# febos/SQUARNA

Measured on AMD Instinct MI355X. Metric: sequences/sec (SRtest150, single-sequence mode), higher is better.
Workload: dtype f64; 1 GPU; SRtest150 if=qf c=nobpp poollim=1000; 8 independent batches in flight per GPU (sq_fold_concurrent, one stream set each), each holding the 219-record set 12 time(s); a step folds all of them; the batches run free inside the timed region (every batch is folded `steps` times back to back, no barrier between the steps: sq_fold_concurrent_n); batches_in_flight=8, sets_per_batch=12, hw_queues=4

## Files before the change

squarna_amd/csrc/sq_lsap.h:

```cpp
#pragma once
#include "sq_match.h"

enum SqLsapForm {
    SQ_LSAP_A,
    SQ_LSAP_B,
    SQ_LSAP_C
};

struct SqLsapLayout {
    double *cost;
    double *u, *v, *spc;
    int32_t *path, *col4row, *row4col, *remaining;
    uint8_t *SR, *SC;
    double *wts;
    uint32_t *mask;
    uint16_t *rowstart;
    uint16_t *pre;
    uint16_t *cids;
    int nw;
    size_t sparse_off;
    size_t lds_end, scratch_end;
};

SQ_HD static inline SqLsapLayout sq_lsap_carve(char *scratch, char *lds, SqLsapForm form, int n, int m)
{
    SqLsapLayout L;
    const size_t N = (size_t)n, M = (size_t)m;
    L.nw = (n + 31) >> 5;
    size_t os = 0, ol = 0;
    sq_take(scratch, os, L.cost, N * N);
    const bool glob = form == SQ_LSAP_C;
    char *const vb = glob ? scratch + os : lds;
    size_t ov = 0;
    sq_take(vb, ov, L.u, N); sq_take(vb, ov, L.v, N); sq_take(vb, ov, L.spc, N);
    sq_take(vb, ov, L.path, N); sq_take(vb, ov, L.col4row, N); sq_take(vb, ov, L.row4col, N); sq_take(vb, ov, L.remaining, N);
    sq_take(vb, ov, L.SR, N); sq_take(vb, ov, L.SC, N);
    if (glob) os += ov;
    ol = ov;
    sq_take(lds, ol, L.wts, M, 16);
    L.sparse_off = (size_t)(reinterpret_cast<char *>(L.wts) - lds);
    sq_take(lds, ol, L.mask, N * L.nw);
    sq_take(lds, ol, L.rowstart, N + 1);
    sq_take(lds, ol, L.pre, N * L.nw, 4);
    sq_take(lds, ol, L.cids, 2 * M, 4);
    L.lds_end = ol; L.scratch_end = os;
    return L;
}

SQ_HD static inline size_t sq_lsap_vec_bytes(int n) { return sq_lsap_carve(nullptr, nullptr, SQ_LSAP_A, n, 0).sparse_off; }
SQ_HD static inline size_t sq_lsap_sparse_bytes(int n, int m)
{
    const SqLsapLayout L = sq_lsap_carve(nullptr, nullptr, SQ_LSAP_A, n, m);
    return L.lds_end - L.sparse_off + 16;
}
SQ_HD static inline size_t sq_lsap_lds_bytes(int n, int m) { return sq_lsap_vec_bytes(n) + sq_lsap_sparse_bytes(n, m) + 64; }
SQ_HD static inline size_t sq_lsap_scratch_bytes(int n) { return sq_lsap_carve(nullptr, nullptr, SQ_LSAP_C, n, 0).scratch_end + 64; }

SQ_HD static inline SqLsapForm sq_lsap_form(int n, int m, size_t lds_bytes)
{
    const bool vec_lds = sq_lsap_vec_bytes(n) + 64 <= lds_bytes;
    const bool mat_lds = vec_lds && m < 32767 && sq_lsap_lds_bytes(n, m) <= lds_bytes;
    return mat_lds ? SQ_LSAP_A : vec_lds ? SQ_LSAP_B : SQ_LSAP_C;
}

struct SqLsapSyncNone {
    SQ_HD void operator()() const {}
    SQ_HD void after_lane0(bool) const {}
};

template <int W, class Sync, class Coop>
SQ_HD_INLINE void sq_lsap_run(const SqLsapLayout &L, SqLsapForm form, int n, int m, const SqMatchEdge *edges, int lane, Sync sync, Coop coop)
{
    const double inf = __builtin_huge_val();
    const bool mat_lds = form == SQ_LSAP_A;
    const int nw = L.nw;
    double *const cost = L.cost, *const u = L.u, *const v = L.v, *const spc = L.spc, *const wts = L.wts;
    int32_t *const path = L.path, *const col4row = L.col4row, *const row4col = L.row4col, *const remaining = L.remaining;
    uint8_t *const SR = L.SR, *const SC = L.SC;
    uint32_t *const mask = L.mask;
    uint16_t *const rowstart = L.rowstart, *const pre = L.pre, *const cids = L.cids;

    if (mat_lds) {
        for (int q = lane; q < n * nw; q += W) mask[q] = 0u;
    } else {
        for (size_t q = lane; q < (size_t)n * n; q += W) cost[q] = 0.0;
    }
    for (int q = lane; q < n; q += W) { u[q] = 0.0; v[q] = 0.0; path[q] = -1; col4row[q] = -1; row4col[q] = -1; }
    sync();
    if (mat_lds) {
        for (int e = lane; e < m; e += W) {
            const SqMatchEdge ed = edges[e];
            wts[e] = ed.weight;
            coop.or_u32(&mask[ed.v * nw + (ed.w >> 5)], 1u << (ed.w & 31));
            coop.or_u32(&mask[ed.w * nw + (ed.v >> 5)], 1u << (ed.v & 31));
        }
        sync();
        const int per = (n + W - 1) / W, r0 = lane * per < n ? lane * per : n, r1 = r0 + per < n ? r0 + per : n;
        int mine = 0;
        for (int r = r0; r < r1; r++) {
            int acc = 0;
            for (int w = 0; w < nw; w++) { pre[r * nw + w] = (uint16_t)acc; acc += __builtin_popcount(mask[r * nw + w]); }
            mine += acc;
        }
        int total = 0;
        int run = coop.excl_scan(mine, total);
        for (int r = r0; r < r1; r++) {
            rowstart[r] = (uint16_t)run;
            run += (int)pre[r * nw + nw - 1] + __builtin_popcount(mask[r * nw + nw - 1]);
        }
        if (lane == W - 1) rowstart[n] = (uint16_t)total;
        sync();
        for (int e = lane; e < m; e += W) {
            const SqMatchEdge ed = edges[e];
            const int a = ed.v, c = ed.w;
            cids[rowstart[a] + pre[a * nw + (c >> 5)] + __builtin_popcount(mask[a * nw + (c >> 5)] & ((1u << (c & 31)) - 1u))] = (uint16_t)e;
            cids[rowstart[c] + pre[c * nw + (a >> 5)] + __builtin_popcount(mask[c * nw + (a >> 5)] & ((1u << (a & 31)) - 1u))] = (uint16_t)e;
        }
    } else {
        for (int e = lane; e < m; e += W) {
            const SqMatchEdge ed = edges[e];
            cost[(size_t)ed.v * n + ed.w] = -ed.weight;
            cost[(size_t)ed.w * n + ed.v] = -ed.weight;
        }
    }
    sync();

    for (int cur = 0; cur < n; cur++) {
        for (int q = lane; q < n; q += W) { remaining[q] = n - q - 1; SR[q] = 0; SC[q] = 0; spc[q] = inf; }
        int i = cur, sink = -1, nrem = n;
        double minval = 0.0;
        sync();
        while (sink == -1) {
            const double ui = u[i];
            const int rs_i = mat_lds ? (int)rowstart[i] : 0;
            double lowest = inf;
            int first = -1, lastun = -1;
            for (int it0 = 0; it0 < nrem; it0 += 3 * W) {
                int jj[3]; bool have[3];
                SQ_UNROLL
                for (int t = 0; t < 3; t++) { const int it = it0 + W * t + lane; have[t] = it < nrem; jj[t] = remaining[have[t] ? it : 0]; }
                uint32_t wd[3]; int pw[3], r4[3]; double vj[3], spj[3], cij[3];
                SQ_UNROLL
                for (int t = 0; t < 3; t++) {
                    const int j = jj[t];
                    vj[t] = v[j]; spj[t] = spc[j]; r4[t] = row4col[j];
                    if (mat_lds) { wd[t] = mask[i * nw + (j >> 5)]; pw[t] = (int)pre[i * nw + (j >> 5)]; cij[t] = 0.0; }
                    else { wd[t] = 0u; pw[t] = 0; cij[t] = cost[(size_t)i * n + j]; }
                }
                if (mat_lds) {
                    int cid[3];
                    SQ_UNROLL
                    for (int t = 0; t < 3; t++) {
                        const int j = jj[t];
                        const bool nz = (wd[t] >> (j & 31)) & 1u;
                        cid[t] = nz ? (int)cids[rs_i + pw[t] + __builtin_popcount(wd[t] & ((1u << (j & 31)) - 1u))] : -1;
                    }
                    SQ_UNROLL
                    for (int t = 0; t < 3; t++) cij[t] = cid[t] >= 0 ? -wts[cid[t]] : 0.0;
                }
                SQ_UNROLL
                for (int t = 0; t < 3; t++) {
                    if (!have[t]) continue;
                    const int it = it0 + W * t + lane, j = jj[t];
                    const double r = minval + cij[t] - ui - vj[t];
                    double sp = spj[t];
                    if (r < sp) { path[j] = i; spc[j] = r; sp = r; }
                    const bool un = r4[t] == -1;
                    if (sp < lowest) { lowest = sp; first = it; lastun = un ? it : -1; }
                    else if (sp == lowest && un) lastun = it;
                }
            }
            double mn = lowest;
            coop.min_plain(mn);
            int f = (lowest == mn && first >= 0) ? first : 0x7fffffff;
            coop.min_i32(f);
            int lu = -((lowest == mn) ? lastun : -1);
            coop.min_i32(lu);
            lu = -lu;
            minval = mn;
            if (mn == inf) { if (lane == 0) SR[i] = 1; sink = -2; break; }
            const int index = lu >= 0 ? lu : f;
            const int j = remaining[index], lastj = remaining[nrem - 1];
            const int owner = row4col[j];
            sync();
            if (lane == 0) { SR[i] = 1; SC[j] = 1; remaining[index] = lastj; }
            nrem--;
            if (owner == -1) sink = j; else i = owner;
            sync.after_lane0(form == SQ_LSAP_C);
        }
        if (sink < 0) break;
        if (lane == 0) u[cur] += minval;
        for (int q = lane; q < n; q += W) {
            if (SR[q] && q != cur) u[q] += minval - spc[col4row[q]];
            if (SC[q]) v[q] -= minval - spc[q];
        }
        sync();
        if (lane == 0) {
            int j = sink;
            for (;;) {
                const int i2 = path[j];
                row4col[j] = i2;
                const int t = col4row[i2]; col4row[i2] = j; j = t;
                if (i2 == cur) break;
            }
        }
        sync();
    }
}
```

squarna_amd/csrc/sq_match.hip:

```cpp
#include <hip/hip_runtime.h>
#include <stdint.h>
#include <math.h>
#include <stdlib.h>
#include <stdio.h>
#include "sq_match.h"
#include "sq_switches.h"
#include "sq_hostflag.h"
#include <vector>
#include <algorithm>
#include "sq_blossom.h"
#include "sq_algo_plan.h"

struct SqLsapBlockSync {
    __device__ void operator()() const { __syncthreads(); }
    __device__ void after_lane0(bool glob) const
    {
        if (glob) __builtin_amdgcn_fence(__ATOMIC_RELEASE, "workgroup");
        __syncthreads();
        if (glob) __builtin_amdgcn_fence(__ATOMIC_ACQUIRE, "workgroup");
    }
};

extern "C" __global__ __launch_bounds__(64) void sq_lsap_kernel(const SqMatchJob *jobs, const SqMatchEdge *edges,
                                                                char *scratch, int32_t *col4row_out, int lds_bytes)
{
    extern __shared__ __attribute__((aligned(16))) char lsap_lds[];
    const SqMatchJob jb = jobs[blockIdx.x];
    const int n = jb.n, m = jb.nedges, lane = threadIdx.x;
    if (n <= 0) return;
    const SqLsapForm form = sq_lsap_form(n, m, (size_t)lds_bytes);
    const SqLsapLayout L = sq_lsap_carve(scratch + jb.scratch_off, lsap_lds, form, n, m);
    sq_lsap_run<64>(L, form, n, m, edges + jb.edge_off, lane, SqLsapBlockSync(), SqCoopWave());
    for (int q = lane; q < n; q += 64) col4row_out[jb.out_off + q] = L.col4row[q];
}

extern "C" __global__ __launch_bounds__(256) void sq_nussinov_kernel(const SqMatchJob *jobs, const SqMatchEdge *edges,
                                                                     const uint8_t *codes, char *scratch,
                                                                     int32_t *pairs_out, int32_t *count_out, int by_pad)
{
    const SqMatchJob jb = jobs[blockIdx.x];
    const int n = jb.n, tid = threadIdx.x, nthr = blockDim.x;
    int32_t *const my_count = count_out + (by_pad ? jb.pad : (int)blockIdx.x);
    if (n < 2) { if (tid == 0) *my_count = 0; return; }
    sq_nussinov_run(sq_nuss_carve(scratch + jb.scratch_off, n, jb.nedges), n, jb.nedges, edges + jb.edge_off, codes + jb.pos_off,
                    pairs_out + 2 * (size_t)jb.out_off, my_count, tid, nthr, [] { __syncthreads(); }, SqCoopWave());
}

template <class Sync>
__device__ __forceinline__ void sq_mwm_one(SqBlossom &bl, char *lds_base, char *wlds, size_t lds_bytes, const SqMatchJob *jp, int row,
                                           const SqMatchEdge *edges, char *scratch, int32_t *mate_out, uint32_t *job_flags,
                                           uint32_t stamp, int lane, Sync wsync)
{
    auto publish = [&]() {
        if (job_flags) {
            const int nw = jp->n > 0 ? 2 * jp->n + 2 : 2;
            sq_host_write_flush(mate_out + jp->out_off + (lane < nw ? nw - 1 - lane : 0));
        }
        wsync();
        if (job_flags && lane == 0) job_flags[row] = stamp;
    };
    const int n = jp->n, m = jp->nedges;
    if (n <= 0) { if (lane == 0) { mate_out[jp->out_off] = 0; mate_out[jp->out_off + 1] = 0; } publish(); return; }
#ifdef SQ_MWM_PROF
    const long long _c0 = clock64(), _w0 = wall_clock64();
#endif
    const size_t ebytes = ((size_t)m * sizeof(SqMatchEdge) + 15) & ~(size_t)15;
    char *gscratch = scratch + jp->scratch_off;
    const bool all_lds = SqBlossom::scratch_bytes(n, m, 1) + ebytes + 16 <= lds_bytes;
    const bool hot_lds = !all_lds && SqBlossom::hot_bytes(n, m, 2) + 16 <= lds_bytes;
    if (all_lds) {
        SqMatchEdge *le = reinterpret_cast<SqMatchEdge *>(wlds);
        for (int e = lane; e < m; e += 64) le[e] = edges[jp->edge_off + e];
        wsync();
#ifdef SQ_MWM_PROF
        const long long _w1 = wall_clock64();
#endif
        if (lane == 0) { bl.init(n, m, le, wlds + ebytes, 1, false); bl.origin = lds_base; }
        wsync();
#ifdef SQ_MWM_PROF
        const long long _w2 = wall_clock64();
#endif
        bl.template build_csr<1>(lane, 64, wsync, SqCoopWave());
#ifdef SQ_MWM_PROF
        const long long _w3 = wall_clock64();
#endif
        bl.template run<1>(lane, 64, wsync, SqCoopWave(), lds_base);
#ifdef SQ_MWM_PROF
        if (lane == 0 && n >= 140) printf("mwm outside: edge load %.0f us, init %.0f, csr %.0f, run %.0f\n", (_w1 - _w0) * 0.01, (_w2 - _w1) * 0.01, (_w3 - _w2) * 0.01, (wall_clock64() - _w3) * 0.01);
#endif
    } else if (hot_lds) {
        if (lane == 0) {
            char *cold = gscratch;
            bl.init(n, m, edges + jp->edge_off, wlds, 2, false, cold, cold + ((SqBlossom::cold_bytes(n, m, 2) + 15) & ~(size_t)15));
            bl.origin = lds_base;
        }
        wsync();
        bl.template build_csr<2>(lane, 64, wsync, SqCoopWave());
        bl.template run<2>(lane, 64, wsync, SqCoopWave(), lds_base);
    }
    if (all_lds || hot_lds) {
        wsync();
        if (!bl.error) {
            for (int q = lane; q < n; q += 64) { mate_out[jp->out_off + q] = bl.mate[q]; mate_out[jp->out_off + n + q] = bl.mord[q]; }
            if (lane == 0) { mate_out[jp->out_off + 2 * n] = bl.stat_pass; mate_out[jp->out_off + 2 * n + 1] = bl.stat_event; }
#ifdef SQ_MWM_PROF
            if (lane == 0 && n >= 140) {
                const long long dc = clock64() - _c0, dw = wall_clock64() - _w0;
                printf("mwm clock: %lld shader cycles in %.0f us -> %.0f MHz\n", dc, dw * 0.01, (double)dc / (dw * 0.01));
            }
#endif
            publish();
            return;
        }
        wsync();
    }
    if (lane == 0) bl.init(n, m, edges + jp->edge_off, gscratch, 0, false);
    wsync();
    bl.template build_csr<0>(lane, 64, wsync, SqCoopWave());
    bl.template run<0>(lane, 64, wsync, SqCoopWave(), nullptr);
    wsync();
    for (int q = lane; q < n; q += 64) { mate_out[jp->out_off + q] = bl.error ? -2 : bl.mate[q]; mate_out[jp->out_off + n + q] = bl.mord[q]; }
    if (lane == 0) { mate_out[jp->out_off + 2 * n] = bl.stat_pass; mate_out[jp->out_off + 2 * n + 1] = bl.stat_event; }
    publish();
}

extern "C" __global__ __launch_bounds__(512, 4) void sq_mwm_kernel(const SqMatchJob *jobs, const int32_t *bin_head,
                                                                const SqMatchEdge *edges, char *scratch, int32_t *mate_out,
                                                                uint32_t *job_flags, uint32_t stamp)
{
    extern __shared__ __attribute__((aligned(16))) char mwm_lds[];
    const int wave = threadIdx.x >> 6, lane = threadIdx.x & 63;
    int row = bin_head[blockIdx.x];
    for (int k = 0; k < wave && row >= 0; k++) row = jobs[row].next;
    if (row < 0) return;
    auto wsync = [] { __builtin_amdgcn_fence(__ATOMIC_SEQ_CST, "workgroup"); __builtin_amdgcn_wave_barrier(); };
    const SqMatchJob *jp = jobs + row;
    const size_t hdr = (sizeof(SqBlossom) + 15) & ~(size_t)15;
    SqBlossom &bl = *reinterpret_cast<SqBlossom *>(mwm_lds + jp->lds_off);
    const size_t lds_bytes = (size_t)jp->lds_bytes > hdr ? (size_t)jp->lds_bytes - hdr : 0;
    sq_mwm_one(bl, mwm_lds, mwm_lds + jp->lds_off + hdr, lds_bytes, jp, row, edges, scratch, mate_out, job_flags, stamp, lane, wsync);
}

extern "C" __global__ __launch_bounds__(64) void sq_mwm_single_kernel(const SqMatchJob *jobs, const SqMatchEdge *edges, char *scratch,
                                                                     int32_t *mate_out, int lds_bytes, uint32_t *job_flags,
                                                                     uint32_t stamp)
{
    __shared__ SqBlossom bl;
    extern __shared__ __attribute__((aligned(16))) char mwm_lds[];
    sq_mwm_one(bl, mwm_lds, mwm_lds, (size_t)lds_bytes, jobs + blockIdx.x, (int)blockIdx.x, edges, scratch, mate_out, job_flags, stamp,
               (int)threadIdx.x, [] { __syncthreads(); });
}

extern "C" __global__ void sq_flag_kernel(uint32_t *flag, uint32_t value)
{
    sq_host_write_flush(flag);
    *flag = value;
}

SqAlgoKnobs sq_algo_knobs(int lsap_classes)
{
    const SqTuning &tu = sq_tuning();
    SqAlgoKnobs kn;
    kn.mwm_classes = tu.mwm_classes; kn.lsap_classes = lsap_classes;
    kn.mwm_bin_waves = tu.mwm_bin_waves; kn.mwm_bin_bytes = tu.mwm_bin_bytes; kn.mwm_all_cap = tu.mwm_all_cap;
    kn.mwm_nolds = tu.mwm_nolds; kn.nuss_threads = tu.nuss_threads;
    return kn;
}

int sq_launch_matching(int algo, const SqMatchJob *h_jobs, int nj, const SqMatchJob *jobs, const SqMatchEdge *edges,
                       size_t nedges, SqMatchEdge *dev_edges, char *d_scr, int32_t *out, int32_t *cnt,
                       const uint8_t *codes, uint32_t *job_flags, uint32_t flag_val, hipStream_t st,
                       SqMatchJob *jobs_rw, int32_t *bin_head, int inflight, const SqAlgoKnobs &kn, bool dump)
{
    int maxn = 0, maxm = 0;
    for (int q = 0; q < nj; q++) { maxn = maxn > h_jobs[q].n ? maxn : h_jobs[q].n; maxm = maxm > h_jobs[q].nedges ? maxm : h_jobs[q].nedges; }
    if (algo == 4) {
        const SqLsapLds P = sq_lsap_launch_lds(h_jobs, nj);
        if (P.need > 64 * 1024) sq_max_dynamic_lds((const void *)sq_lsap_kernel, (int)SQ_LSAP_LDS_CAP);
        hipLaunchKernelGGL(sq_lsap_kernel, dim3(nj), dim3(64), P.lds, st, jobs, edges, d_scr, out, (int)P.lds);
    } else if (algo == 2) {
        const int nthr = sq_nussinov_threads(h_jobs, nj, maxn, inflight, kn);
        hipLaunchKernelGGL(sq_nussinov_kernel, dim3(nj), dim3(nthr), 0, st, jobs, edges, codes, d_scr, out, cnt, jobs_rw ? 1 : 0);
    } else {
        const SqMwmPlan P = sq_mwm_plan(h_jobs, jobs_rw, nj, bin_head, inflight, kn, dump);
        const size_t lds = P.lds;
        sq_max_dynamic_lds((const void *)sq_mwm_kernel, 156 * 1024);
        if (!P.all_in_lds && dev_edges != edges) {
            hipError_t e = hipMemcpyAsync(dev_edges, edges, nedges * sizeof(SqMatchEdge), hipMemcpyHostToDevice, st);
            if (e != hipSuccess) return (int)e;
            edges = dev_edges;
        }
        if (P.waves == 1) {
            sq_max_dynamic_lds((const void *)sq_mwm_single_kernel, 156 * 1024);
            const size_t one = lds > sq_blossom_hdr() ? lds - sq_blossom_hdr() : 0;
            hipLaunchKernelGGL(sq_mwm_single_kernel, dim3(nj), dim3(64), one, st, jobs, edges, d_scr, out, (int)one, job_flags, flag_val);
        } else
            hipLaunchKernelGGL(sq_mwm_kernel, dim3(P.nbins), dim3(64 * P.waves), lds, st, jobs, bin_head, edges, d_scr, out, job_flags, flag_val);
    }
    return (int)hipGetLastError();
}
```

squarna_amd/csrc/sq_nussinov.h:

```cpp
#pragma once
#include "sq_match.h"

struct SqNussLayout {
    double *cs;
    int32_t *ck;
    int32_t *col_off, *cursor;
    double *D;
    int32_t *K;
    uint8_t *has;
    int32_t *cur, *nxt;
    size_t lists_end, lists_room;
    size_t end;
};

SQ_HD static inline SqNussLayout sq_nuss_carve(char *scratch, int n, int m)
{
    SqNussLayout L;
    const size_t N = (size_t)n, M = (size_t)m;
    size_t o = 0;
    sq_take(scratch, o, L.cs, M); sq_take(scratch, o, L.ck, M); sq_take(scratch, o, L.col_off, N + 1); sq_take(scratch, o, L.cursor, N);
    L.lists_end = o;
    o = L.lists_room = N * N * sizeof(double);
    sq_take(scratch, o, L.D, N * N);
    sq_take(scratch, o, L.K, N * N);
    sq_take(scratch, o, L.has, (N * N + 15) & ~(size_t)15);
    sq_take(scratch, o, L.cur, 2 * (N + 2)); sq_take(scratch, o, L.nxt, 2 * (N + 2));
    L.end = o;
    return L;
}

static inline size_t sq_nussinov_scratch_bytes(int n) { return sq_nuss_carve(nullptr, n, 0).end + 64; }

template <class Sync, class Coop>
SQ_HD_INLINE void sq_nussinov_run(const SqNussLayout &L, int n, int m, const SqMatchEdge *edges, const uint8_t *cd, int32_t *out,
                                  int32_t *count, int tid, int nthr, Sync sync, Coop coop)
{
    double *const cs = L.cs;
    int32_t *const ck = L.ck, *const col_off = L.col_off, *const cursor = L.cursor;
    uint8_t *const has = L.has;
    for (size_t q = tid; q < (size_t)n * n; q += nthr) has[q] = 0;
    for (int q = tid; q < n; q += nthr) L.D[(size_t)q * n + q] = 0.0;
    for (int q = tid; q <= n; q += nthr) col_off[q] = 0;
    sync();
    for (int e = tid; e < m; e += nthr) coop.add_i32(&col_off[edges[e].w + 1], 1);
    sync();
    if (tid == 0) for (int j = 0; j < n; j++) col_off[j + 1] += col_off[j];
    sync();
    for (int q = tid; q < n; q += nthr) cursor[q] = col_off[q];
    sync();
    for (int e = tid; e < m; e += nthr) {
        const SqMatchEdge ed = edges[e];
        const int pos = coop.fetch_add_i32(&cursor[ed.w], 1);
        ck[pos] = ed.v; cs[pos] = -ed.weight;
    }
    sync();
    for (int j = tid; j < n; j += nthr) {
        const int a = col_off[j], b = col_off[j + 1];
        for (int x = a + 1; x < b; x++) {
            const int kk = ck[x]; const double vv = cs[x];
            int y = x - 1;
            while (y >= a && ck[y] > kk) { ck[y + 1] = ck[y]; cs[y + 1] = cs[y]; y--; }
            ck[y + 1] = kk; cs[y + 1] = vv;
        }
    }
    sync();
    double *const Dc = L.D;
    int32_t *const Kc = L.K;
    for (int j = 1; j < n; j++) {
        const int x0 = col_off[j], x1 = col_off[j + 1];
        const double *const dprevcol = Dc + (size_t)(j - 1) * n;
        for (int i = tid; i < j; i += nthr) {
            int bestk = -1; double best = 1e9;
            for (int x = x0; x < x1; x += 4) {
                int kk[4]; double d1[4], d2[4], cw[4]; bool ok[4];
                SQ_UNROLL
                for (int t = 0; t < 4; t++) { const int k = ck[x + t < x1 ? x + t : x]; kk[t] = x + t < x1 ? k : 0x7fffffff; }
                SQ_UNROLL
                for (int t = 0; t < 4; t++) {
                    ok[t] = kk[t] >= i && kk[t] < j - 1;
                    d1[t] = 0.0; d2[t] = 0.0; cw[t] = 0.0;
                    if (ok[t]) {
                        if (kk[t] > i) d1[t] = Dc[(size_t)(kk[t] - 1) * n + i];
                        d2[t] = dprevcol[kk[t] + 1];
                        cw[t] = cs[x + t];
                    }
                }
                SQ_UNROLL
                for (int t = 0; t < 4; t++)
                    if (ok[t]) {
                        const double sc = d1[t] + d2[t] + cw[t];
                        if (sc < best) { bestk = kk[t]; best = sc; }
                    }
                if (kk[3] >= j - 1) break;
            }
            const double dprev = dprevcol[i];
            const bool take = best <= dprev;
            Kc[(size_t)j * n + i] = take ? bestk : -2;
            Dc[(size_t)j * n + i] = take ? best : dprev;
        }
        sync();
    }
    if (tid == 0) {
        const int minloop = 3;
        int32_t *const cur = L.cur, *const nxt = L.nxt;
        uint8_t *inq = has;
        int qn = 1, np = 0;
        cur[0] = 0; cur[1] = n - 1;
        auto sep = [&](int p) { return cd[p] == 26 || cd[p] == 27; };
        auto anysep = [&](int a, int b) { for (int x = a; x < b; x++) if (x >= 0 && x < n && sep(x)) return true; return false; };
        while (qn) {
            int nn = 0;
            for (int t = 0; t < qn; t++) {
                const int i = cur[2 * t], j = cur[2 * t + 1];
                if (i < 0 || j < 0 || i >= n || j >= n) continue;
                auto push = [&](int a, int b) {
                    if (!inq[(size_t)a * n + b]) { inq[(size_t)a * n + b] = 1; nxt[2 * nn] = a; nxt[2 * nn + 1] = b; nn++; }
                };
                const int kk = Kc[(size_t)j * n + i];
                if (kk != -2) {
                    const int k = kk;
                    if (((k - 1) - i > minloop) || ((k - 1) - i > 0 && anysep(i + 1, k - 1))) push(i, k - 1);
                    if (((j - 1) - (k + 1) > minloop) || ((j - 1) - (k + 1) > 0 && anysep(k + 2, j - 1))) push(k + 1, j - 1);
                    out[2 * np] = k; out[2 * np + 1] = j; np++;
                } else {
                    if (((j - 1) - i > minloop) || ((j - 1) - i > 0 && anysep(i + 1, j - 1))) push(i, j - 1);
                }
            }
            for (int t = 0; t < nn; t++) inq[(size_t)nxt[2 * t] * n + nxt[2 * t + 1]] = 0;
            for (int t = 0; t < 2 * nn; t++) cur[t] = nxt[t];
            qn = nn;
        }
        *count = np;
    }
}
```

Baseline: 658,500 seq/s.

## Add single-wave Nussinov DP with register-resident columns and tail-sized LSAP scan

Adds a wave-only Nussinov path for sequences of at most 192 residues. Each lane keeps its rows' previous-column D values in registers and shares them with readlane, so the per-column block barrier becomes wave-level waits. The column list prefix sum now uses a cooperative scan, and the backtrack drops the has-matrix clear and its dedup check. Separately, the LSAP scan picks a 1-, 2- or 3-slot variant for the last chunk so lanes do not load entries past the end. The cost is more register pressure from the per-lane arrays and more code variants; the dedup removal assumes duplicate intervals cannot occur.

```diff
diff --git a/squarna_amd/csrc/sq_lsap.h b/squarna_amd/csrc/sq_lsap.h
--- a/squarna_amd/csrc/sq_lsap.h
+++ b/squarna_amd/csrc/sq_lsap.h
@@ -68,6 +68,8 @@
     SQ_HD void after_lane0(bool) const {}
 };
 
+template <int N> struct SqLsapSlots { static constexpr int value = N; };
+
 template <int W, class Sync, class Coop>
 SQ_HD_INLINE void sq_lsap_run(const SqLsapLayout &L, SqLsapForm form, int n, int m, const SqMatchEdge *edges, int lane, Sync sync, Coop coop)
 {
@@ -135,31 +137,32 @@
             const int rs_i = mat_lds ? (int)rowstart[i] : 0;
             double lowest = inf;
             int first = -1, lastun = -1;
-            for (int it0 = 0; it0 < nrem; it0 += 3 * W) {
-                int jj[3]; bool have[3];
+            auto scan = [&](auto ns, int it0) {
+                constexpr int NS = decltype(ns)::value;
+                int jj[NS]; bool have[NS];
                 SQ_UNROLL
-                for (int t = 0; t < 3; t++) { const int it = it0 + W * t + lane; have[t] = it < nrem; jj[t] = remaining[have[t] ? it : 0]; }
-                uint32_t wd[3]; int pw[3], r4[3]; double vj[3], spj[3], cij[3];
+                for (int t = 0; t < NS; t++) { const int it = it0 + W * t + lane; have[t] = it < nrem; jj[t] = remaining[have[t] ? it : 0]; }
+                uint32_t wd[NS]; int pw[NS], r4[NS]; double vj[NS], spj[NS], cij[NS];
                 SQ_UNROLL
-                for (int t = 0; t < 3; t++) {
+                for (int t = 0; t < NS; t++) {
                     const int j = jj[t];
                     vj[t] = v[j]; spj[t] = spc[j]; r4[t] = row4col[j];
                     if (mat_lds) { wd[t] = mask[i * nw + (j >> 5)]; pw[t] = (int)pre[i * nw + (j >> 5)]; cij[t] = 0.0; }
                     else { wd[t] = 0u; pw[t] = 0; cij[t] = cost[(size_t)i * n + j]; }
                 }
                 if (mat_lds) {
-                    int cid[3];
+                    int cid[NS];
                     SQ_UNROLL
-                    for (int t = 0; t < 3; t++) {
+                    for (int t = 0; t < NS; t++) {
                         const int j = jj[t];
                         const bool nz = (wd[t] >> (j & 31)) & 1u;
                         cid[t] = nz ? (int)cids[rs_i + pw[t] + __builtin_popcount(wd[t] & ((1u << (j & 31)) - 1u))] : -1;
                     }
                     SQ_UNROLL
-                    for (int t = 0; t < 3; t++) cij[t] = cid[t] >= 0 ? -wts[cid[t]] : 0.0;
+                    for (int t = 0; t < NS; t++) cij[t] = cid[t] >= 0 ? -wts[cid[t]] : 0.0;
                 }
                 SQ_UNROLL
-                for (int t = 0; t < 3; t++) {
+                for (int t = 0; t < NS; t++) {
                     if (!have[t]) continue;
                     const int it = it0 + W * t + lane, j = jj[t];
                     const double r = minval + cij[t] - ui - vj[t];
@@ -169,6 +172,12 @@
                     if (sp < lowest) { lowest = sp; first = it; lastun = un ? it : -1; }
                     else if (sp == lowest && un) lastun = it;
                 }
+            };
+            for (int it0 = 0; it0 < nrem; it0 += 3 * W) {
+                const int left = nrem - it0;
+                if (left <= W) scan(SqLsapSlots<1>(), it0);
+                else if (left <= 2 * W) scan(SqLsapSlots<2>(), it0);
+                else scan(SqLsapSlots<3>(), it0);
             }
             double mn = lowest;
             coop.min_plain(mn);
diff --git a/squarna_amd/csrc/sq_match.hip b/squarna_amd/csrc/sq_match.hip
--- a/squarna_amd/csrc/sq_match.hip
+++ b/squarna_amd/csrc/sq_match.hip
@@ -42,8 +42,16 @@
     const int n = jb.n, tid = threadIdx.x, nthr = blockDim.x;
     int32_t *const my_count = count_out + (by_pad ? jb.pad : (int)blockIdx.x);
     if (n < 2) { if (tid == 0) *my_count = 0; return; }
-    sq_nussinov_run(sq_nuss_carve(scratch + jb.scratch_off, n, jb.nedges), n, jb.nedges, edges + jb.edge_off, codes + jb.pos_off,
-                    pairs_out + 2 * (size_t)jb.out_off, my_count, tid, nthr, [] { __syncthreads(); }, SqCoopWave());
+    const SqNussLayout L = sq_nuss_carve(scratch + jb.scratch_off, n, jb.nedges);
+    if (nthr == SqNussLanesWave::kLanes && sq_nuss_wave_fits(n)) {
+        SqNussLanesWave ln;
+        ln.lane_ = tid;
+        sq_nussinov_wave_run(L, n, jb.nedges, edges + jb.edge_off, codes + jb.pos_off, pairs_out + 2 * (size_t)jb.out_off, my_count, ln,
+                             [] { __syncthreads(); }, SqCoopWave(), SqNussNoProbe());
+        return;
+    }
+    sq_nussinov_run(L, n, jb.nedges, edges + jb.edge_off, codes + jb.pos_off, pairs_out + 2 * (size_t)jb.out_off, my_count, tid, nthr,
+                    [] { __syncthreads(); }, SqCoopWave());
 }
 
 template <class Sync>
diff --git a/squarna_amd/csrc/sq_nussinov.h b/squarna_amd/csrc/sq_nussinov.h
--- a/squarna_amd/csrc/sq_nussinov.h
+++ b/squarna_amd/csrc/sq_nussinov.h
@@ -31,22 +31,30 @@
 
 static inline size_t sq_nussinov_scratch_bytes(int n) { return sq_nuss_carve(nullptr, n, 0).end + 64; }
 
-template <class Sync, class Coop>
-SQ_HD_INLINE void sq_nussinov_run(const SqNussLayout &L, int n, int m, const SqMatchEdge *edges, const uint8_t *cd, int32_t *out,
-                                  int32_t *count, int tid, int nthr, Sync sync, Coop coop)
+template <bool kCoopScan, class Sync, class Coop>
+SQ_HD_INLINE void sq_nuss_build_lists(const SqNussLayout &L, int n, int m, const SqMatchEdge *edges, int tid, int nthr, Sync sync, Coop coop)
 {
     double *const cs = L.cs;
     int32_t *const ck = L.ck, *const col_off = L.col_off, *const cursor = L.cursor;
-    uint8_t *const has = L.has;
-    for (size_t q = tid; q < (size_t)n * n; q += nthr) has[q] = 0;
-    for (int q = tid; q < n; q += nthr) L.D[(size_t)q * n + q] = 0.0;
     for (int q = tid; q <= n; q += nthr) col_off[q] = 0;
     sync();
     for (int e = tid; e < m; e += nthr) coop.add_i32(&col_off[edges[e].w + 1], 1);
     sync();
-    if (tid == 0) for (int j = 0; j < n; j++) col_off[j + 1] += col_off[j];
-    sync();
-    for (int q = tid; q < n; q += nthr) cursor[q] = col_off[q];
+    if (kCoopScan) {
+        int run = 0;
+        for (int q0 = 0; q0 < n; q0 += nthr) {
+            const int q = q0 + tid;
+            const int c = q < n ? col_off[q + 1] : 0;
+            int total;
+            const int ex = coop.excl_scan(c, total);
+            if (q < n) { col_off[q + 1] = run + ex + c; cursor[q] = run + ex; }
+            run += total;
+        }
+    } else {
+        if (tid == 0) for (int j = 0; j < n; j++) col_off[j + 1] += col_off[j];
+        sync();
+        for (int q = tid; q < n; q += nthr) cursor[q] = col_off[q];
+    }
     sync();
     for (int e = tid; e < m; e += nthr) {
         const SqMatchEdge ed = edges[e];
@@ -64,6 +72,50 @@
         }
     }
     sync();
+}
+
+template <class Probe>
+SQ_HD_INLINE void sq_nuss_backtrack(const SqNussLayout &L, int n, const uint8_t *cd, int32_t *out, int32_t *count, Probe probe)
+{
+    const int minloop = 3;
+    const int32_t *const Kc = L.K;
+    int32_t *cur = L.cur, *nxt = L.nxt;
+    int qn = 1, np = 0;
+    cur[0] = 0; cur[1] = n - 1;
+    auto sep = [&](int p) { return cd[p] == 26 || cd[p] == 27; };
+    auto anysep = [&](int a, int b) { for (int x = a; x < b; x++) if (x >= 0 && x < n && sep(x)) return true; return false; };
+    while (qn) {
+        int nn = 0;
+        for (int t = 0; t < qn; t++) {
+            const int i = cur[2 * t], j = cur[2 * t + 1];
+            if (i < 0 || j < 0 || i >= n || j >= n) continue;
+            auto push = [&](int a, int b) { probe(a, b, nxt, nn); nxt[2 * nn] = a; nxt[2 * nn + 1] = b; nn++; };
+            const int kk = Kc[(size_t)j * n + i];
+            if (kk != -2) {
+                const int k = kk;
+                if (((k - 1) - i > minloop) || ((k - 1) - i > 0 && anysep(i + 1, k - 1))) push(i, k - 1);
+                if (((j - 1) - (k + 1) > minloop) || ((j - 1) - (k + 1) > 0 && anysep(k + 2, j - 1))) push(k + 1, j - 1);
+                out[2 * np] = k; out[2 * np + 1] = j; np++;
+            } else {
+                if (((j - 1) - i > minloop) || ((j - 1) - i > 0 && anysep(i + 1, j - 1))) push(i, j - 1);
+            }
+        }
+        int32_t *const was = cur; cur = nxt; nxt = was;
+        qn = nn;
+    }
+    *count = np;
+}
+
+struct SqNussNoProbe { SQ_HD void operator()(int, int, const int32_t *, int) const {} };
+
+template <class Sync, class Coop>
+SQ_HD_INLINE void sq_nussinov_run(const SqNussLayout &L, int n, int m, const SqMatchEdge *edges, const uint8_t *cd, int32_t *out,
+                                  int32_t *count, int tid, int nthr, Sync sync, Coop coop)
+{
+    double *const cs = L.cs;
+    int32_t *const ck = L.ck, *const col_off = L.col_off;
+    for (int q = tid; q < n; q += nthr) L.D[(size_t)q * n + q] = 0.0;
+    sq_nuss_build_lists<false>(L, n, m, edges, tid, nthr, sync, coop);
     double *const Dc = L.D;
     int32_t *const Kc = L.K;
     for (int j = 1; j < n; j++) {
@@ -100,36 +152,149 @@
         }
         sync();
     }
-    if (tid == 0) {
-        const int minloop = 3;
-        int32_t *const cur = L.cur, *const nxt = L.nxt;
-        uint8_t *inq = has;
-        int qn = 1, np = 0;
-        cur[0] = 0; cur[1] = n - 1;
-        auto sep = [&](int p) { return cd[p] == 26 || cd[p] == 27; };
-        auto anysep = [&](int a, int b) { for (int x = a; x < b; x++) if (x >= 0 && x < n && sep(x)) return true; return false; };
-        while (qn) {
-            int nn = 0;
-            for (int t = 0; t < qn; t++) {
-                const int i = cur[2 * t], j = cur[2 * t + 1];
-                if (i < 0 || j < 0 || i >= n || j >= n) continue;
-                auto push = [&](int a, int b) {
-                    if (!inq[(size_t)a * n + b]) { inq[(size_t)a * n + b] = 1; nxt[2 * nn] = a; nxt[2 * nn + 1] = b; nn++; }
-                };
-                const int kk = Kc[(size_t)j * n + i];
-                if (kk != -2) {
-                    const int k = kk;
-                    if (((k - 1) - i > minloop) || ((k - 1) - i > 0 && anysep(i + 1, k - 1))) push(i, k - 1);
-                    if (((j - 1) - (k + 1) > minloop) || ((j - 1) - (k + 1) > 0 && anysep(k + 2, j - 1))) push(k + 1, j - 1);
-                    out[2 * np] = k; out[2 * np + 1] = j; np++;
-                } else {
-                    if (((j - 1) - i > minloop) || ((j - 1) - i > 0 && anysep(i + 1, j - 1))) push(i, j - 1);
+    if (tid == 0) sq_nuss_backtrack(L, n, cd, out, count, SqNussNoProbe());
+}
+
+#ifndef SQ_NUSS_WAVE_SLOTS
+#define SQ_NUSS_WAVE_SLOTS 3
+#endif
+#define SQ_NUSS_WAVE_ROWS (64 * SQ_NUSS_WAVE_SLOTS)
+#ifndef SQ_NUSS_WAVE_TRIP
+#define SQ_NUSS_WAVE_TRIP 4
+#endif
+
+SQ_HD static inline bool sq_nuss_wave_fits(int n) { return n >= 2 && n <= SQ_NUSS_WAVE_ROWS; }
+
+struct SqNussLanesOne {
+    static constexpr int kLanes = 1, kOwn = SQ_NUSS_WAVE_ROWS;
+    double prev[kOwn];
+    int lane() const { return 0; }
+    double of_row(int k) const { return prev[k]; }
+    int pass(int v, int) const { return v; }
+    double pass(double v, int) const { return v; }
+    int same(int v) const { return v; }
+    void arrived() const {}
+    void publish() const {}
+};
+#ifdef __HIPCC__
+struct SqNussLanesWave {
+    static constexpr int kLanes = 64, kOwn = SQ_NUSS_WAVE_SLOTS;
+    double prev[kOwn];
+    int lane_;
+    __device__ int lane() const { return lane_; }
+    __device__ int pass(int v, int l) const { return __builtin_amdgcn_readlane(v, l); }
+    __device__ double pass(double v, int l) const
+    {
+        return __hiloint2double(__builtin_amdgcn_readlane(__double2hiint(v), l), __builtin_amdgcn_readlane(__double2loint(v), l));
+    }
+    __device__ int same(int v) const { return __builtin_amdgcn_readfirstlane(v); }
+    __device__ void arrived() const { __builtin_amdgcn_s_waitcnt(0x0F70); }
+    __device__ double of_row(int k) const
+    {
+        double v = pass(prev[0], k & 63);
+        SQ_UNROLL
+        for (int s = 1; s < kOwn; s++) { const double w = pass(prev[s], k & 63); if ((k >> 6) == s) v = w; }
+        return v;
+    }
+    __device__ void publish() const
+    {
+        __builtin_amdgcn_fence(__ATOMIC_RELEASE, "workgroup");
+        __syncthreads();
+        __builtin_amdgcn_fence(__ATOMIC_ACQUIRE, "workgroup");
+    }
+};
+#endif
+
+template <class Lanes>
+SQ_HD_INLINE void sq_nuss_wave_entries(const SqNussLayout &L, int n, int j, int cnt, int lk, double ls, double (&best)[Lanes::kOwn],
+                                       int (&bestk)[Lanes::kOwn], const Lanes &ln)
+{
+    constexpr int kLanes = Lanes::kLanes, kOwn = Lanes::kOwn, kTrip = SQ_NUSS_WAVE_TRIP;
+    const int lane = ln.lane();
+    const double *const Dc = L.D;
+    for (int e = 0; e < cnt; e += kTrip) {
+        int kk[kTrip]; double d1[kTrip][kOwn];
+        SQ_UNROLL
+        for (int t = 0; t < kTrip; t++) kk[t] = e + t < cnt ? ln.pass(lk, e + t < kLanes ? e + t : 0) : 0x7fffffff;
+        SQ_UNROLL
+        for (int t = 0; t < kTrip; t++) {
+            SQ_UNROLL
+            for (int s = 0; s < kOwn; s++) {
+                const int i = s * kLanes + lane;
+                d1[t][s] = 0.0;
+                if (kk[t] < j - 1 && s * kLanes < kk[t] - 1) d1[t][s] = Dc[(size_t)(kk[t] - 1) * n + (i < kk[t] - 1 ? i : kk[t] - 1)];
+            }
+        }
+        ln.arrived();
+        SQ_UNROLL
+        for (int t = 0; t < kTrip; t++) {
+            if (kk[t] < j - 1) {
+                const double d2 = ln.of_row(kk[t] + 1);
+                const double cw = ln.pass(ls, e + t < kLanes ? e + t : 0);
+                SQ_UNROLL
+                for (int s = 0; s < kOwn; s++) {
+                    const int i = s * kLanes + lane;
+                    const double sc = (kk[t] - 1 > i ? d1[t][s] : 0.0) + d2 + cw;
+                    if (kk[t] >= i && sc < best[s]) { bestk[s] = kk[t]; best[s] = sc; }
                 }
             }
-            for (int t = 0; t < nn; t++) inq[(size_t)nxt[2 * t] * n + nxt[2 * t + 1]] = 0;
-            for (int t = 0; t < 2 * nn; t++) cur[t] = nxt[t];
-            qn = nn;
-        }
-        *count = np;
-    }
-}
+        }
+    }
+}
+
+template <class Lanes>
+SQ_HD_INLINE void sq_nuss_wave_column(const SqNussLayout &L, int n, int j, int x0, int x1, int lk, double ls, int &ahead, Lanes &ln)
+{
+    constexpr int kLanes = Lanes::kLanes, kOwn = Lanes::kOwn;
+    const int lane = ln.lane();
+    double *const Dc = L.D;
+    int32_t *const Kc = L.K;
+    int bestk[kOwn]; double best[kOwn];
+    SQ_UNROLL
+    for (int s = 0; s < kOwn; s++) { bestk[s] = -1; best[s] = 1e9; }
+    sq_nuss_wave_entries(L, n, j, x1 - x0 < kLanes ? x1 - x0 : kLanes, lk, ls, best, bestk, ln);
+    for (int xb = x0 + kLanes; xb < x1; xb += kLanes) {
+        const int mk = xb + lane < x1 ? L.ck[xb + lane] : 0x7fffffff;
+        const double ms = xb + lane < x1 ? L.cs[xb + lane] : 0.0;
+        sq_nuss_wave_entries(L, n, j, x1 - xb < kLanes ? x1 - xb : kLanes, mk, ms, best, bestk, ln);
+    }
+    ln.arrived();
+    ahead = ln.same(ahead);
+    SQ_UNROLL
+    for (int s = 0; s < kOwn; s++) {
+        const int i = s * kLanes + lane;
+        if (i < j) {
+            const double dprev = ln.prev[s];
+            const bool take = best[s] <= dprev;
+            const double d = take ? best[s] : dprev;
+            Kc[(size_t)j * n + i] = take ? bestk[s] : -2;
+            Dc[(size_t)j * n + i] = d;
+            ln.prev[s] = d;
+        }
+    }
+}
+
+template <class Lanes, class Sync, class Coop, class Probe>
+SQ_HD_INLINE void sq_nussinov_wave_run(const SqNussLayout &L, int n, int m, const SqMatchEdge *edges, const uint8_t *cd, int32_t *out,
+                                       int32_t *count, Lanes &ln, Sync sync, Coop coop, Probe probe)
+{
+    constexpr int kLanes = Lanes::kLanes, kOwn = Lanes::kOwn;
+    const int lane = ln.lane();
+    const int32_t *const col_off = L.col_off;
+    sq_nuss_build_lists<true>(L, n, m, edges, lane, kLanes, sync, coop);
+    SQ_UNROLL
+    for (int s = 0; s < kOwn; s++) ln.prev[s] = 0.0;
+    int xa = ln.same(col_off[1]), xb = ln.same(col_off[2]), xc = ln.same(col_off[3 < n ? 3 : n]);
+    int lk = xa + lane < xb ? L.ck[xa + lane] : 0x7fffffff;
+    double ls = xa + lane < xb ? L.cs[xa + lane] : 0.0;
+    ln.arrived();
+    for (int j = 1; j < n; j++) {
+        const int nlk = xb + lane < xc ? L.ck[xb + lane] : 0x7fffffff;
+        const double nls = xb + lane < xc ? L.cs[xb + lane] : 0.0;
+        int xd = col_off[j + 3 < n ? j + 3 : n];
+        sq_nuss_wave_column(L, n, j, xa, xb, lk, ls, xd, ln);
+        xa = xb; xb = xc; xc = xd; lk = nlk; ls = nls;
+    }
+    ln.publish();
+    if (lane == 0) sq_nuss_backtrack(L, n, cd, out, count, probe);
+}
```

After: 625,700 seq/s. 0.95x the previous value.
